# DINT-NSDI24/DINT

Hardware: AMD Instinct MI355X
Metric: Mtxn/s + p50/p99 batch latency, TATP (higher is better)
Workload: dtype u64

## Files before the change

### dint_amd/csrc/dint_kernels.h

```cpp
#pragma once
#include <hip/hip_runtime.h>
#include <stdint.h>

#include "dint_device.h"

struct dint_dev_stats {
  unsigned long long bad_requests;
  unsigned long long missing_keys;
  unsigned long long foreign_requests;
  unsigned long long pool_exhausted;
  unsigned long long route_overflow;
  unsigned long long big_bin_requests;
  unsigned long long late_requests;
  unsigned long long late_items[3];
};

struct dint_kv_sets {
  uint32_t *ctl[3] = {nullptr, nullptr, nullptr};
  uint32_t *pub[3] = {nullptr, nullptr, nullptr};
  uint32_t *bin_cnt[2] = {nullptr, nullptr};
  uint4 *kbins[2] = {nullptr, nullptr};
  uint4 *ovl[2] = {nullptr, nullptr};
  uint32_t *bigrdy = nullptr;
  uint64_t *sbx = nullptr;
  uint64_t pass_no = 0;
};

#define DINT_KV_HOTPUB_WORDS (3u * DINT_KV_BIGQ_MAX)
#define DINT_KV_SBX_WORDS 48u

struct dint_scratch {
  uint32_t *bin_cnt;
  uint64_t *bins;
  dint_dev_stats *stats;
  uint32_t *blk_cnt;
  uint32_t *blk_pub;
  uint32_t *blk_pub_next;
  uint32_t *big;
  uint32_t *big_next;
  uint32_t *bin_off;
  uint4 *ovl;
  uint64_t *ovf;
  uint64_t *ovf2;
  uint4 *kbins = nullptr;
  uint64_t kbins_slots = 0;
  uint4 *bigq = nullptr;
// ... 61 lines not shown
```

### dint_amd/csrc/dint_kv.h

```cpp
#pragma once
#include <cstdlib>
#include <utility>
#include <vector>

#include "dint_kernels.h"
#include "dint_kv_core.h"
#include "state_image.h"

#define DINT_KV_MAX_TABLES 5
#define DINT_KV_CTL_BYTES (64 + 24 * KV_NLISTS)
#define DINT_KV_TRACE_WORDS ((size_t)DINT_KV_PMAX * 16 + 16 * 8192)
#define DINT_KV_LOAD_OP 0xF0u

struct kv_dev {
  kv_tab tab[DINT_KV_MAX_TABLES];
  dint_mod mod[DINT_KV_MAX_TABLES];
  dint_mod lockmod[DINT_KV_MAX_TABLES];
  uint32_t gk_base[DINT_KV_MAX_TABLES];
  uint32_t n_tables;
  uint32_t shard_index, shard_count;
  uint32_t same_key;
};

struct dint_kv_knobs {
  uint32_t coarse_load = 512;
  uint32_t cap = 0;
  uint32_t lcap = 1024;
  uint32_t cap_mult = 64;
  uint32_t rpt = 0;
  uint32_t no_bm = 0;
  uint32_t hot_min = 0;
  uint32_t no_split = 0;
  uint32_t split_min = 65;
  uint32_t split_target = 384;
  uint32_t one_big_kernel = 0;
  uint32_t workers = 96;
  uint32_t part_first = 0;
  uint32_t sb_split_min = 65;
  uint32_t sb_npmax = 128;
  uint32_t sb_workers = 130;
  uint32_t sb_late_grid = 32;
  uint32_t residency = 0;
  uint32_t no_fuse = 0;
  uint32_t no_ahead = 0;
  uint32_t late_grid = 8;
  uint32_t exp_no_late = 0;
  uint32_t late_fat = 0;
  uint32_t late_big = 0;
};

struct dint_kv {
  uint32_t workload = 0;
  uint32_t n_tables = 0;
  uint32_t val_size = 0;
  int force_rounds = 0;
  uint64_t hash_size[DINT_KV_MAX_TABLES] = {0, 0, 0, 0, 0};
  kv_dev h{};
  kv_dev *d_dev = nullptr;
  uint8_t *d_ctl = nullptr;
  uint64_t *d_trace = nullptr;
  size_t entry_bytes[DINT_KV_MAX_TABLES] = {0, 0, 0, 0, 0};
  dint_kv_knobs knobs;
};

static inline uint32_t dint_kv_cap_mult() {
  const char *v = getenv("DINT_KV_CAP_MULT");
  const unsigned long m = v && *v ? strtoul(v, nullptr, 10) : 64ul;
  return (uint32_t)(m < 2 ? 2 : m > 256 ? 256 : m);
}
int dint_kv_create(dint_kv *kv, uint32_t workload, uint64_t n_rows, dint_shard shard, uint32_t pool_entries = 0,
// ... 135 lines not shown
```

### dint_amd/csrc/engine.hip

```cpp
#include <hip/hip_runtime.h>

#include <algorithm>
#include <cstdarg>
#include <cstdio>
#include <cstdlib>
#include <cstring>
#include <mutex>
#include <string>
#include <vector>

#include "../../include/dint_abi.h"
#include "dint_kernels.h"
#include "dint_kv.h"
#include "dint_populate.h"
#include "state_rehash.h"
#include "state_stats.h"

void dint_launch_lock_stage(uint32_t workload, int stage, const void *d_req, void *d_rep, uint32_t n, uint2 *table, dint_mod slots,
                            dint_shard shard, dint_scratch s, hipStream_t st, const dint_view &view);
bool dint_launch_lock_fused(uint32_t workload, void *d_rep, uint32_t n, uint2 *table, dint_mod slots, dint_shard shard, dint_scratch s,
                            const dint_view &view, const void *next_req, void *next_rep, uint32_t next_n, dint_scratch sn,
                            const dint_view &next_view, hipStream_t st);

namespace {
// ... 671 lines not shown
      TRY(dev_alloc((void **)&e->scratch.kvs.ovl[1], (size_t)e->pass_max * sizeof(uint4) * 2, false));
      TRY(dev_alloc((void **)&e->scratch.kvs.bigrdy, (size_t)DINT_KV_BIGQ_MAX * sizeof(uint32_t)));
      if (wl == DINT_WL_SMALLBANK)
        TRY(dev_alloc((void **)&e->scratch.kvs.sbx, (size_t)DINT_KV_BIGQ_MAX * DINT_KV_SBX_WORDS * sizeof(uint64_t), false));
    } else {
      TRY(dev_alloc((void **)&e->scratch.bins, (size_t)DINT_KV_PMAX * DINT_KV_BINCAP * sizeof(uint64_t), false));
      if (!getenv("DINT_LOCK_NO_DIRECT")) {
        e->scratch.kbins_slots = 1024ull * 65536ull;
        TRY(dev_alloc((void **)&e->scratch.kbins, (size_t)e->scratch.kbins_slots * sizeof(uint64_t), false));
      }
    }
    TRY(dev_alloc((void **)&e->scratch.blk_pub, 3 * 1024 * sizeof(uint32_t)));
    e->scratch.blk_pub_next = e->scratch.blk_pub + 1024;
    TRY(dev_alloc((void **)&e->scratch.big, 2 * (4 + DINT_KV_PMAX) * sizeof(uint32_t)));
    e->scratch.big_next = e->scratch.big + (4 + DINT_KV_PMAX);
    if (is_kv)
      for (int k = 0; k < 3; k++) { e->scratch.kvs.ctl[k] = e->scratch.big + 16 * k; e->scratch.kvs.pub[k] = e->scratch.blk_pub + 1024 * k; }
    TRY(dev_alloc((void **)&e->scratch.bin_off, DINT_KV_PMAX * sizeof(uint32_t)));
    TRY(hipMemset(e->scratch.bin_off, 0xFF, DINT_KV_PMAX * sizeof(uint32_t)) == hipSuccess ? 0 : fail(DINT_EHIP, "hipMemset"));
    TRY(dev_alloc((void **)&e->scratch.ovl, (size_t)e->pass_max * sizeof(uint4) * (is_kv ? 2 : 1), false));
    TRY(dev_alloc((void **)&e->scratch.ovf, (size_t)e->pass_max * sizeof(uint64_t), false));
    if (is_kv) {
      TRY(dev_alloc((void **)&e->scratch.ovf2, (size_t)e->pass_max * sizeof(uint64_t), false));
      e->scratch.kvs.bin_cnt[0] = e->scratch.bin_cnt; e->scratch.kvs.kbins[0] = e->scratch.kbins; e->scratch.kvs.ovl[0] = e->scratch.ovl;
    }
    if ((e->cfg.workload == DINT_WL_FASST || e->cfg.workload == DINT_WL_2PL) && getenv("DINT_KV_TRACE")) {
      TRY(dev_alloc((void **)&e->kv.d_trace, (size_t)DINT_KV_TRACE_WORDS * 8, true));
      e->scratch.lock_trace = e->kv.d_trace;
    }
  } else {
    TRY(dev_alloc((void **)&e->scratch.blk_pub, 2 * (1024 + 16) * sizeof(uint32_t)));
    e->scratch.blk_pub_next = e->scratch.blk_pub + (1024 + 16);
  }
  TRY(slot_alloc(e, 0));
  if (hipHostMalloc((void **)&e->h_pinned, (size_t)e->pass_max * e->msg_size + 64, hipHostMallocDefault) != hipSuccess ||
      hipHostMalloc((void **)&e->h_pool, 64, hipHostMallocDefault) != hipSuccess) {
    dint_engine_destroy(e);
    return fail(DINT_ENOMEM, "hipHostMalloc");
  }
  *e->h_pool = 0;

  if (wl == DINT_WL_FASST || wl == DINT_WL_2PL) {
    e->n_slots = cfg->n_slots ? cfg->n_slots : 36000000ull;
    if (e->n_slots > 0xFFFFFFF0ull) { dint_engine_destroy(e); return fail(DINT_EINVAL, "n_slots too large"); }
    e->slots_mod = dint_make_mod(e->n_slots);
    e->n_local_slots = (e->n_slots + e->shard.count - 1) / e->shard.count;
// ... 30 lines not shown
  for (auto &sl : e->slot)
    if (sl.deliver_to && sl.h_rep) { memcpy(sl.deliver_to, sl.h_rep, sl.deliver_bytes); sl.deliver_to = nullptr; }
  for (hipEvent_t ev : e->timer.ev) hipEventDestroy(ev);
  for (void *p : e->snap) hipFree(p);
  hipFree(e->scratch.bin_cnt);
  hipFree(e->scratch.bins);
  hipFree(e->scratch.kbins);
  hipFree(e->scratch.bigq);
  hipFree(e->scratch.hotpub);
  hipFree(e->scratch.lateq);
  hipFree(e->scratch.kvs.bin_cnt[1]);
  hipFree(e->scratch.kvs.kbins[1]);
  hipFree(e->scratch.kvs.ovl[1]);
  hipFree(e->scratch.kvs.bigrdy);
  hipFree(e->scratch.kvs.sbx);
  hipFree(e->scratch.stats);
  hipFree(e->scratch.blk_cnt);
  hipFree(std::min(e->scratch.blk_pub, e->scratch.blk_pub_next));
  hipFree(std::min(e->scratch.big, e->scratch.big_next));
  hipFree(e->scratch.bin_off);
  hipFree(e->scratch.ovl);
  hipFree(e->scratch.ovf);
  hipFree(e->scratch.ovf2);
  if (e->scratch.lock_trace) { hipFree(e->scratch.lock_trace); e->kv.d_trace = nullptr; }
  for (auto &sl : e->slot) {
    hipFree(sl.d_req);
    hipFree(sl.d_rep);
    if (sl.h_req) hipHostFree(sl.h_req);
    if (sl.h_rep) hipHostFree(sl.h_rep);
    if (sl.h2d) hipEventDestroy(sl.h2d);
    if (sl.comp) hipEventDestroy(sl.comp);
    if (sl.done) hipEventDestroy(sl.done);
  }
  hipFree(std::min(e->route.blk, e->route.blk_next));
  if (e->h_pinned) hipHostFree(e->h_pinned);
  if (e->h_pool) hipHostFree(e->h_pool);
  if (e->ev_order) hipEventDestroy(e->ev_order);
  if (e->ev_route_order) hipEventDestroy(e->ev_route_order);
  if (e->ev_wait) hipEventDestroy(e->ev_wait);
  if (e->ev_signal) hipEventDestroy(e->ev_signal);
  if (e->s_h2d && e->s_h2d != e->stream) hipStreamDestroy(e->s_h2d);
  if (e->s_d2h && e->s_d2h != e->stream) hipStreamDestroy(e->s_d2h);
  lock_pipe_destroy(e);
  replay_free(e);
  state_free(e);
  hipFree(e->tstats.part); hipFree(e->tstats.out);
// ... 1217 lines not shown
```

### dint_amd/csrc/k_kv.hip

```cpp
#include "k_kv_dev.h"

dint_kv_fmt dint_kv_format(uint32_t workload) {
  switch (workload) {
    case DINT_WL_STORE: return {53, 0, 0xFFFFFFFFu, 1, 9, 49, 40};
    case DINT_WL_TATP: return {55, 1, 2, 3, 11, 51, 40};
    default: return {23, 1, 2, 3, 11, 19, 8};
  }
}


static inline uint32_t kv_pick_coarse(uint32_t n, uint32_t load) {
  uint64_t c = ((uint64_t)n + load - 1) / load;
  if (c < 1) c = 1;
  if (c > DINT_KV_CMAX) c = DINT_KV_CMAX;
  return (uint32_t)c;
}
static uint32_t kv_env(const char *name, uint32_t dflt) {
  const char *v = getenv(name);
  return v && *v ? (uint32_t)strtoul(v, nullptr, 10) : dflt;
}
static dint_kv_knobs kv_read_knobs() {
  dint_kv_knobs k;
  k.coarse_load = std::min(8192u, std::max(64u, kv_env("DINT_KV_COARSE_LOAD", KVB_T)));
  k.cap = kv_env("DINT_KV_CAP", 0);
  k.lcap = std::min(KVR_LCAP, kv_env("DINT_KV_LCAP", KVR_LCAP));
  k.cap_mult = dint_kv_cap_mult();
  k.rpt = kv_env("DINT_KV_RPT", 0);
  k.no_bm = kv_env("DINT_KV_NO_BM", 0);
  k.hot_min = kv_env("DINT_KV_HOT_MIN", 0);
  k.no_split = kv_env("DINT_KV_NO_SPLIT", 0);
  k.split_min = std::max(65u, kv_env("DINT_KV_SPLIT_MIN", 65u));
  k.split_target = std::min(448u, std::max(8u, kv_env("DINT_KV_SPLIT_TARGET", 384u)));
  k.one_big_kernel = kv_env("DINT_KV_ONE_BIG_KERNEL", 0);
  k.no_ahead = kv_env("DINT_KV_NO_AHEAD", 0);
  k.no_fuse = kv_env("DINT_KV_NO_FUSE", 0);
  k.sb_split_min = kv_env("DINT_KV_SB_SPLIT_MIN", 65u);
  k.sb_late_grid = std::max(1u, std::min(KVB_GRID, kv_env("DINT_KV_SB_LATE_GRID", 32u)));
  k.sb_npmax = std::max(2u, std::min(KSB_NPMAX, kv_env("DINT_KV_SB_NPMAX", 128u)));
  k.sb_workers = kv_env("DINT_KV_SB_WORKERS", k.sb_npmax + 2u);
  if (k.sb_workers) k.sb_workers = std::max(k.sb_workers, k.sb_npmax + 2u);
  k.workers = std::min(1024u, std::max(KVR_NPMAX + 2u, kv_env("DINT_KV_WORKERS", KVW_GRID)));
  k.part_first = kv_env("DINT_KV_PART_FIRST", 0) & 1u;
  k.late_grid = std::min(KVB_GRID, std::max(1u, kv_env("DINT_KV_LATE_GRID", 8u)));
  k.late_big = kv_env("DINT_KV_LATE_BIG", 0);
  k.exp_no_late = kv_env("DINT_EXP_NO_LATE", 0);
  k.late_fat = kv_env("DINT_KV_LATE_FAT", 0);
  return k;
}

static inline bool kv_uses_hot(const dint_kv &kv, int load_mode) {
  return kv.workload != DINT_WL_SMALLBANK && !(kv.force_rounds & 3) && !load_mode && !kv.knobs.no_split;
}
bool dint_kv_one_launch(const dint_kv &kv, int load_mode) {
  return kv_uses_hot(kv, load_mode) && !kv.knobs.one_big_kernel && !kv.knobs.no_fuse;
}
bool dint_kv_ahead_ok(const dint_kv &kv, int load_mode) {
  if (kv.workload == DINT_WL_SMALLBANK) return !load_mode && !kv.knobs.no_ahead && !kv.knobs.no_fuse;
  return kv_uses_hot(kv, load_mode) && !kv.knobs.one_big_kernel && !kv.knobs.no_ahead;
}

static void kv_fill_pass(kv_pass_args &A, const void *d_req, void *d_rep, uint32_t n, const dint_kv &kv, dint_log log,
                         const dint_scratch &s, int load_mode, const dint_view &view, uint32_t tile) {
  const dint_kv_knobs &K = kv.knobs;
  const uint32_t C = kv_pick_coarse(n, K.coarse_load);
  const uint32_t mean = (n + C - 1) / C;
  uint32_t cap = K.cap_mult * mean + 64;
  cap = std::min(cap, (uint32_t)(s.kbins_slots / C));
  cap = std::max(1u, K.cap ? std::min(cap, K.cap) : cap);
  A.req = (const uint8_t *)d_req; A.rep = (uint8_t *)d_rep; A.n = n;
  A.n_tiles = (n + tile - 1) / tile;
  A.kv = kv.d_dev; A.log = log; A.cut = kv_make_cut(C, n); A.cap = cap;
  A.lcap = K.lcap;
  const uint64_t pn = s.kvs.pass_no;
  A.pno = (uint32_t)(pn & 1u);
  A.bin_cnt = s.kvs.bin_cnt[pn & 1]; A.kbins = s.kvs.kbins[pn & 1]; A.ovl = s.kvs.ovl[pn & 1];
  A.big = s.kvs.ctl[pn % 3]; A.big_z = s.kvs.ctl[(pn + 2) % 3];
  A.blk_pub = s.kvs.pub[pn % 3]; A.blk_pub_z = s.kvs.pub[(pn + 2) % 3];
  A.bigrdy = s.kvs.bigrdy;
  A.ovf = s.ovf; A.ovf2 = s.ovf2; A.stats = s.stats;
  A.bigq = s.bigq;
  A.hotpub = s.hotpub;
  A.lateq = s.lateq;
  A.seq = s.pass_seq ? s.pass_seq : 1u;
  A.inv_n = n > 1 ? (uint32_t)((1ull << 32) / n) : 0xFFFFFFFFu;
  A.load_mode = load_mode;
  A.force_flags = kv.force_rounds | (K.no_bm ? 4 : 0) | (int)(K.hot_min << 8);
  A.split_min = kv_uses_hot(kv, load_mode) ? K.split_min : 0xFFFFFFFFu;
  A.split_target = K.split_target;
  A.np_max = KVR_NPMAX;
  A.sb_pieces = 0;
  A.sbx = s.kvs.sbx;
  if (kv.workload == DINT_WL_SMALLBANK && K.sb_split_min && s.kvs.sbx && !(kv.force_rounds & 3) && !load_mode && !K.no_split) {
    A.split_min = std::max(8u, K.sb_split_min);
    A.np_max = K.sb_npmax;
    A.sb_pieces = 1;
  }
  A.has_log = kv.workload != DINT_WL_STORE;
  A.trace = kv.d_trace;
  A.V = view;
}

extern template int kv_piece_residency<DINT_WL_STORE>(int);
extern template int kv_piece_residency<DINT_WL_TATP>(int);
extern template int kv_piece_residency<DINT_WL_SMALLBANK>(int);
extern template void launch_kv_passes<DINT_WL_STORE>(kv_multi_args &, uint32_t, uint32_t, hipStream_t, hipEvent_t *, const dint_kv_knobs &, bool, const kv_multi_args *, uint32_t);
extern template void launch_kv_passes<DINT_WL_TATP>(kv_multi_args &, uint32_t, uint32_t, hipStream_t, hipEvent_t *, const dint_kv_knobs &, bool, const kv_multi_args *, uint32_t);
extern template void launch_kv_passes<DINT_WL_SMALLBANK>(kv_multi_args &, uint32_t, uint32_t, hipStream_t, hipEvent_t *, const dint_kv_knobs &, bool, const kv_multi_args *, uint32_t);

static inline uint32_t kv_pick_rpt(uint32_t n_total, const dint_kv_knobs &K) {
  if (K.rpt == 1 || K.rpt == 2 || K.rpt == 4) return K.rpt;
  return n_total >= 1024u * 1024u ? 4u : n_total >= 256u * 1024u ? 2u : 1u;
// ... 292 lines not shown
```

### dint_amd/csrc/k_kv_dev.h

```cpp
#pragma once
#include <algorithm>
#include <cstdlib>
#include <cstring>
#include <utility>
#include <vector>

#include "../../include/dint_abi.h"
#include "dint_kv.h"
#define KVB_SORT_INLINE
#include "dint_bins.h"

template <int WL> struct Fmt;
template <> struct Fmt<DINT_WL_STORE> {
  static constexpr uint32_t MSG = 53, TYPE = 0, KEY = 1, VAL = 9, VER = 49, VS = 40;
  static constexpr bool HAS_TABLE = false;
  static constexpr uint32_t TABLE = 0;
};
template <> struct Fmt<DINT_WL_TATP> {
  static constexpr uint32_t MSG = 55, TYPE = 1, KEY = 3, VAL = 11, VER = 51, VS = 40;
  static constexpr bool HAS_TABLE = true;
  static constexpr uint32_t TABLE = 2;
};
template <> struct Fmt<DINT_WL_SMALLBANK> {
  static constexpr uint32_t MSG = 23, TYPE = 1, KEY = 3, VAL = 11, VER = 19, VS = 8;
// ... 102 lines not shown
}

struct kv_pass_args {
  const uint8_t *req;
  uint8_t *rep;
  uint32_t n, n_tiles;
  const kv_dev *kv;
  dint_log log;
  kv_cut cut;
  uint32_t cap;
  uint32_t lcap;
  uint32_t *bin_cnt;
  uint4 *kbins;
  uint32_t *big, *big_z;
  uint32_t *blk_pub, *blk_pub_z;
  uint32_t *bigrdy;
  uint64_t *sbx;
  uint32_t np_max;
  uint32_t sb_pieces;
  uint32_t pno;
  uint4 *ovl;
  uint64_t *ovf;
  uint64_t *ovf2;
  uint4 *bigq;
  unsigned long long *hotpub;
  uint4 *lateq;
  uint32_t split_min;
  uint32_t split_target;
  uint32_t inv_n;
  uint32_t seq;
  dint_dev_stats *stats;
  int load_mode, force_flags;
  uint32_t has_log;
  uint64_t *trace;
  dint_view V;
};
struct kv_multi_args { kv_pass_args e[DINT_KV_MULTI_MAX]; };

__device__ static inline uint64_t u4_key(const uint4 &r) { return ((uint64_t)r.y << 32) | r.x; }
__device__ static inline uint64_t u4_meta(const uint4 &r) { return ((uint64_t)r.w << 32) | r.z; }

template <uint32_t TB, uint32_t... Ks>
__device__ __forceinline__ static void kv_copy_tile(const uint4 *__restrict__ s, uint4 *__restrict__ d, uint32_t nv, uint32_t t,
                                                    std::integer_sequence<uint32_t, Ks...>) {
  const uint4 v[] = {s[min(t + Ks * TB, nv - 1)]...};
  ((d[min(t + Ks * TB, nv - 1)] = v[Ks]), ...);
}

template <int RPT, uint32_t TB = KV_TB>
struct kv_part_lds {
  uint32_t Hc[DINT_KV_CMAX];
  uint32_t Sov[2];
  uint32_t Stile;
  uint32_t Swl[TB / 64 * RPT], Swp[TB / 64];
};
template <int WL, int RPT, uint32_t TB = KV_TB>
__device__ __forceinline__ static void kv_part_body(const kv_pass_args &A, kv_part_lds<RPT, TB> &S, bool first_block) {
  using F = Fmt<WL>;
  constexpr uint32_t T = TB * RPT, NWV = TB / 64;
  auto &Hc = S.Hc; auto &Sov = S.Sov; auto &Stile = S.Stile; auto &Swl = S.Swl; auto &Swp = S.Swp;
// ... 1884 lines not shown
#undef KVB_STAMP
}

#define KVR_LCAP 1024u
#define KVR_F 64u
#define KVR_NPMAX 64u
struct kvr_lds {
  uint4 rec[KVR_LCAP];
  uint32_t hist[KVR_F];
  uint32_t cur[KVR_F];
  uint32_t off[KVR_F + 1];
  uint32_t bigoff[KVR_F];
  uint2 chs[KVR_F];
  uint32_t nch;
  uint32_t cflag[KVR_F];
  uint64_t ckey[KVR_F], hrec[KVR_F];
};
__device__ static inline uint32_t kv_piece_of(uint32_t idx, uint32_t np, uint32_t inv_n) {
  const uint32_t p = (uint32_t)(((uint64_t)idx * np * inv_n) >> 32);
  return p < np ? p : np - 1;
}
#define KVQ_W 3u
enum : uint32_t { KVQ_SUB = 0, KVQ_PIECE = 1, KVQ_REM = 2, KVQ_SOLO = 3 };

__device__ static inline void kv_list_items(const kv_pass_args &A, uint32_t b, const kvr_lds &L, const uint2 *Sbig) {
  const uint32_t t = threadIdx.x & 63u;
  const uint2 bs = Sbig[t];
  uint32_t target = A.split_target;
  if (A.V.seg_cap) {
    uint32_t live = t < A.V.n_seg ? min(A.V.seg_cap, *(const uint32_t *)(A.V.cnt + (size_t)t * A.V.cnt_stride)) : 0u, tot;
    (void)wave_excl_scan_u32(live, &tot);
    if (tot < A.n) target = max(8u, (uint32_t)(((uint64_t)target * max(tot, 1u)) / A.n));
  }
  const uint32_t np0 = (bs.y + target - 1) / target;
  const bool hot = bs.y >= A.split_min && np0 <= A.np_max;
  const uint32_t np = hot ? np0 : 0u;
  const uint32_t nent = bs.y ? (np > 1 ? np + 1 : 1u) : 0u;
  uint32_t tot, at = wave_excl_scan_u32(nent, &tot);
  uint32_t base = 0;
  if (t == 0 && tot) base = atomicAdd(&A.big[3], tot);
  base = (uint32_t)__builtin_amdgcn_readfirstlane((int)base);
  at += base;
  const uint32_t bin = b + A.cut.P * t;
  if (nent && !hot) {
    kv_st_agent(A.bigq + KVQ_W * (size_t)at, make_uint4(bin, bs.x, bs.y, KVQ_SUB));
  } else if (nent) {
    uint64_t hk = L.ckey[t], hr = L.hrec[t];
    if (A.sb_pieces) {
      using F = Fmt<DINT_WL_SMALLBANK>;
      const uint32_t sh_g = 16 + A.cut.ibits;
      uint64_t smp[8];
#pragma unroll
      for (uint32_t j = 0; j < 8; j++) smp[j] = kv_ld_agent(&A.ovf[bs.x + (uint32_t)(((uint64_t)(2 * j + 1) * bs.y) >> 4)]);
      uint32_t best = 0, bj = 0;
#pragma unroll
      for (uint32_t j = 0; j < 8; j++) {
// ... 442 lines not shown
    for (uint32_t wv = 0; wv < KVB_W; wv++) {
      uint64_t mm = H.Bl[wv];
      if (wv * 64 > P) break;
      if (wv == (P >> 6)) mm &= (2ull << (P & 63)) - 1ull;
      if (mm) Gs = wv * 64 + 63 - (uint32_t)__clzll((long long)mm);
    }
    Ge = h;
    for (uint32_t wv = P >> 6; wv < KVB_W && Ge == h; wv++) {
      uint64_t mm = H.Bl[wv];
      if (wv == (P >> 6)) mm &= ~((2ull << (P & 63)) - 1ull);
      if (mm) Ge = wv * 64 + (uint32_t)__ffsll((unsigned long long)mm) - 1;
    }
  }
  auto rest = [&](uint32_t lo, uint32_t len) -> int {
    const uint32_t c_rem = h - len;
    if (c_rem == 0) return 0;
    __syncthreads();
    if (valid && (t < lo || t >= lo + len)) H.rem[t < lo ? t : t - len] = w;
    if (t >= c_rem) H.rem[t] = ~0ull;
    __builtin_amdgcn_fence(__ATOMIC_SEQ_CST, "workgroup");
    if (kv_rem_chunks<WL>(rep, cut2, kv, d.x, H.rem, c_rem, H, stats, force_rounds, V, true)) return 0;
    if (ovf2 && t < c_rem) {
      const uint64_t sw = H.rem[t];
      ovf2[d.y + t] = ((sw >> sh_g) << sh_g) | ((uint64_t)((uint32_t)(sw >> 7) & idx_mask) << 16) | ((uint32_t)sw & 0x7Fu) | (((uint32_t)(sw >> sh_k) & 511u) << 7);
    }
    __builtin_amdgcn_fence(__ATOMIC_SEQ_CST, "workgroup");
    *src = 1; *off = d.y; *cnt = c_rem;
    return 1;
  };
  auto phases = [&]() -> int {
    if (!kv_group_phases<WL>(rep, cut2, kv, d.x, H.all, Gs, Ge, H, stats, V)) return 1;
    return rest(Gs, Ge - Gs);
  };
  if (L <= 64) {
    if (ttr && t == 0) ttr[30] = (uint64_t)(d.w & 0xFFFFu) | (1ull << 17) | ((uint64_t)L << 20) | ((uint64_t)h << 32);
    if (Ge - Gs <= 64) return kv_rem_chunks<WL>(rep, cut2, kv, d.x, H.all, h, H, stats, force_rounds, V, true) ? 0 : 1;
    return phases();
  }
  const uint64_t hw = H.all[P];
  const uint32_t hq = pay_q((uint32_t)hw & 0x7Fu);
  const bool v = valid && t >= P && t < P + L;
  const uint32_t my_idx = (uint32_t)(w >> 7) & idx_mask, my_type = valid ? pay_type((uint32_t)w & 0x7Fu) : 0xFFu;
  if (valid && !v && (w >> sh_g) == (hw >> sh_g) && (kv_struct_op<WL>(my_type) || (kv_lock_op<WL>(my_type) && pay_q((uint32_t)w & 0x7Fu) == hq))) atomicOr(&H.bad, kv_struct_op<WL>(my_type) ? 1u : 2u);
  const uint64_t my_key = v ? ld_u64(rep + dint_view_off(V, my_idx, F::MSG) + F::KEY) : 0;
  if (t == P) H.hkey = my_key;
  const bool setop = v && is_set(my_type), insop = v && is_ins(my_type), delop = v && is_del(my_type);
  const bool lk = v && kv_lock_op<WL>(my_type), aq = v && WL == DINT_WL_TATP && my_type == 1;
// ... 154 lines not shown
    const bool same_g = k < h && (r >> sh_g) == (hrec >> sh_g), same = same_g && pay_kh(pay) == hkh;
    if (same_g && !same) {
      H.nbr = 1;
      if (kv_struct_op<WL>(type) || (kv_lock_op<WL>(type) && pay_q(pay) == hq)) H.bad = 1;
    }
    if (do_piece) {
      const bool mine = same && (np == 1 || kv_piece_of(ridx, np, inv_n) == j);
      const bool really = mine && ld_u64(rep + dint_view_off(V, ridx, F::MSG) + F::KEY) == hkey;
      if (mine && !really) H.bad = 1;
      const uint64_t mm = __ballot(really), ms = __ballot(same);
      uint32_t at = 0;
      if (lane == 0 && mm) at = atomicAdd(&H.nhot, (uint32_t)__popcll(mm));
      if (lane == 0 && ms) atomicAdd(&H.nsame, (uint32_t)__popcll(ms));
      at = (uint32_t)__builtin_amdgcn_readfirstlane((int)at) + (uint32_t)__popcll(mm & lanemask_lt());
      if (really && at < KVB_T) { H.key[at] = (ridx << 9) | at; H.typ[at] = (uint8_t)(type & 0xFFu); }
    }
    if (do_rem) {
      const bool other = k < h && !same;
      const uint64_t mm = __ballot(other);
      uint32_t at = 0;
      if (lane == 0 && mm) at = atomicAdd(&H.nrem, (uint32_t)__popcll(mm));
      at = (uint32_t)__builtin_amdgcn_readfirstlane((int)at) + (uint32_t)__popcll(mm & lanemask_lt());
      if (other) {
        ovf2[d.y + at] = r;
        if (at < KVB_T) H.rem[at] = r;
      }
    }
    if (solo && k < h && k < KVB_T) H.all[k] = r;
  }
  __syncthreads();
  const uint32_t c_rem = do_rem ? H.nrem : 0u, nbr = H.nbr;
  if (solo && H.nhot <= 64 && h <= KVB_T) {
    if (ttr && t == 0) ttr[30] = (uint64_t)(d.w & 0xFFFFu) | (1ull << 17) | ((uint64_t)H.nhot << 20) | ((uint64_t)h << 32);
    if (kv_rem_chunks<WL>(rep, cut2, kv, d.x, H.all, h, H, stats, force_rounds, V)) return 0;
    *src = 0; *off = d.y; *cnt = h;
    return 1;
  }
  const uint32_t c = do_piece ? H.nhot : 0u;
  if (t == 0 && c > KVB_T) H.bad = 1;
  const uint32_t nsib = np > 1 ? np + (nbr ? 1u : 0u) : 1u;
  const bool voting = do_piece || (nbr && np > 1);
  kv_hdr Hd;
  kv_tab tb0;
  uint64_t bucket0 = 0;
  uint32_t table0 = 0;
  const bool locator = t == 0 && c != 0;
  if (locator) {
// ... 128 lines not shown
        }
        st_u32(msg + F::VER, ver0 + nw_before + wr_below);
      }
      msg[F::TYPE] = (uint8_t)code;
    }
    if (found && nw_all && (int)j == jw && (int)t == lw_tot) {
      kv_copy_words(row, rep + dint_view_off(V, my_idx, F::MSG) + F::VAL, F::VS);
      KV_ST(uint32_t, &kv_entry_hdr(tb, bucket, H.link)->ver[H.slot], ver0 + nw_all);
    }
    if (WL == DINT_WL_TATP && t == 0) {
      if ((int)j == jl && la_fin >= 0 && (uint32_t)la_fin != la0) KV_ST(uint8_t, kv_entry_ptr(tb, bucket, KV_INLINE) + KV_LOCKB_OFF + hq, (uint8_t)la_fin);
      if (!found && wr_tot) atomicAdd(&stats->missing_keys, (unsigned long long)wr_tot);
    }
  }
  if (c_rem == 0) return 0;
  __builtin_amdgcn_fence(__ATOMIC_SEQ_CST, "workgroup");
  if (c_rem <= KVB_T && kv_rem_chunks<WL>(rep, cut2, kv, d.x, H.rem, c_rem, H, stats, force_rounds, V)) return 0;
  __builtin_amdgcn_fence(__ATOMIC_SEQ_CST, "workgroup");
  *src = 1; *off = d.y; *cnt = c_rem;
  return 1;
}

template <int WL>
__device__ __forceinline__ static void kv_serial_group(uint8_t *rep, const kv_cut cut2, const kv_dev *kv, uint32_t bin, const uint64_t *R, uint32_t Gs,
                                                       uint32_t Ge, kvh_lds &H, dint_dev_stats *__restrict__ stats, const dint_view V) {
  using F = Fmt<WL>;
  const uint32_t t = threadIdx.x, n = Ge - Gs;
  const uint32_t sh_g = 16 + cut2.ibits, idx_mask = (uint32_t)((1ull << cut2.ibits) - 1ull);
  __syncthreads();
  {
    const uint64_t w = t < n ? R[Gs + t] : 0;
    const uint32_t idx = (uint32_t)(w >> 7) & idx_mask, pay = (uint32_t)w & 0x7Fu;
    H.key[t] = t < n ? (idx << 9) | t : 0xFFFFFFFFu;
    H.typ[t] = (uint8_t)(pay_type(pay) & 0xFFu);
    H.qq[t] = (uint8_t)pay_q(pay);
  }
  __syncthreads();
  kvb_sort_blocked_u32<1>(H.key, KVB_T);
  if (t == 0) {
    const uint32_t gk = kv_cut_gk((uint32_t)(R[Gs] >> sh_g), bin, cut2), table = kv_table_of(kv, gk);
    const uint64_t bucket = (uint64_t)(gk - kv->gk_base[table]);
    for (uint32_t p = 0; p < n; p++) {
      const uint32_t sk = H.key[p], slot = sk & 511u;
      kv_do_request<WL>(rep + dint_view_off(V, sk >> 9, F::MSG), H.typ[slot], table, H.qq[slot], bucket, kv, stats);
      __builtin_amdgcn_fence(__ATOMIC_SEQ_CST, "workgroup");
    }
// ... 44 lines not shown
      return;
    }
    if (force_rounds || !kv_group_phases<WL>(rep, cut2, kv, bin, H.all, Gs, Gs + len, H, stats, V))
      kv_serial_group<WL>(rep, cut2, kv, bin, H.all, Gs, Gs + len, H, stats, V);
    __syncthreads();
    const bool mv = t >= Gs + len && t < m;
    const uint64_t mw = mv ? H.all[t] : 0;
    __syncthreads();
    if (mv) H.all[t - len] = mw;
    if (t >= m - len && t < m) H.all[t] = ~0ull;
    m -= len;
    if (m == 0) return;
  }
}
#define KVL_RANGES 4096u
struct kvl_lds {
  uint32_t pre[KVL_RANGES];
  uint32_t wsum[KVB_W];
  uint32_t cnt;
};
template <int WL>
__device__ __forceinline__ static void kv_late_item(const kv_pass_args &A, const kv_cut cut2, const kv_dev *kv, const uint4 d, kvh_lds &H, kvl_lds &L) {
  const uint32_t t = threadIdx.x, lane = t & 63, wave = t >> 6;
  const uint64_t *__restrict__ recs = (d.w ? (const uint64_t *)A.ovf2 : A.ovf) + d.y;
  const uint32_t cnt = d.z, bin = d.x;
  if (cnt == 0) return;
  if (cnt <= KVB_T) {
    __syncthreads();
    H.all[t] = t < cnt ? kv_sort_key(recs[t], cut2) : ~0ull;
    kv_late_stretch<WL>(A.rep, cut2, kv, bin, cnt, H, A.stats, A.force_flags & 1, A.V);
    return;
  }
  const uint32_t rw = (A.n + KVL_RANGES - 1) / KVL_RANGES;
  __syncthreads();
  for (uint32_t k = t; k < KVL_RANGES; k += KVB_T) L.pre[k] = 0;
  __syncthreads();
  for (uint32_t k = t; k < cnt; k += KVB_T) atomicAdd(&L.pre[min(KVL_RANGES - 1, kv_rec_idx(recs[k], cut2) / rw)], 1u);
  __syncthreads();
  {
    constexpr uint32_t PT = KVL_RANGES / KVB_T;
    uint32_t v[PT], sum = 0;
#pragma unroll
    for (uint32_t k = 0; k < PT; k++) { v[k] = L.pre[t * PT + k]; sum += v[k]; }
    uint32_t tot, base = wave_excl_scan_u32(sum, &tot);
    if (lane == 0) L.wsum[wave] = tot;
    __syncthreads();
    for (uint32_t w = 0; w < wave; w++) base += L.wsum[w];
// ... 315 lines not shown
      }
      st_u32(msg + F::VER, ver0 + nw_before + wr_below);
    } else if (get && my_type != 17u) {
      miss = 1;
    }
    msg[F::TYPE] = (uint8_t)code;
  }
  {
    const uint64_t mm = __ballot(miss != 0);
    if (lane == 0 && mm) atomicAdd(&stats->missing_keys, (unsigned long long)__popcll(mm));
  }
  if (found && nw_all && (int)j == jw && (int)t == lw_tot) {
    uint8_t *row = kv_entry_ptr(tb, bucket, H.link) + KV_VAL_OFF + H.slot * F::VS;
    KV_ST(uint32_t, row, ld_u32(msg + F::VAL));
    KV_ST(uint32_t, row + 4, ld_u32(msg + F::VAL + 4));
    KV_ST(uint32_t, &kv_entry_hdr(tb, bucket, H.link)->ver[H.slot], ver0 + nw_all);
  }
  return done();
}

static_assert(sizeof(kvb_lds) + KVB_BM_BYTES + sizeof(kv_dev) <= 160 * 1024, "k_kv_big must fit the 160 KB of LDS of a gfx950 CU");
static_assert(sizeof(kvb_lds) + (KV_HOT_BM ? KV_HOT_BM_W * 10 : 16) + sizeof(kv_dev) <= 160 * 1024, "k_kv_big must fit the 160 KB of LDS of a gfx950 CU");
#define KVW_GRID 96u
template <int WL>
__device__ __forceinline__ static void kv_hot_role(const kv_pass_args &A, kv_dev &Skv, uint8_t *Lraw, uint32_t &Stk, uint32_t bx, uint32_t by) {
  const uint32_t t = threadIdx.x;
  if (t < sizeof(kv_dev) / 4) ((uint32_t *)&Skv)[t] = ((const uint32_t *)A.kv)[t];
  __syncthreads();
  kv_dev_pend_set(Skv, A.pno);
  kv_cut cut2 = A.cut;
  cut2.P = A.cut.P * KVR_F;
  uint64_t *tr = A.trace ? A.trace + 2048 * 32 + 32 * (size_t)(by * KVB_GRID + bx) : nullptr;
  for (bool first = true;; first = false) {
    __syncthreads();
    if (t == 0) {
      const uint32_t i = atomicAdd(&A.big[4], 1u);
      uint32_t got = KV_NONE;
      for (uint32_t spins = 0; i < DINT_KV_BIGQ_MAX; spins++) {
        if (__hip_atomic_load(&A.bigrdy[i], __ATOMIC_RELAXED, __HIP_MEMORY_SCOPE_AGENT) == A.seq) { got = i; break; }
        if (__hip_atomic_load(&A.big[6], __ATOMIC_RELAXED, __HIP_MEMORY_SCOPE_AGENT) >= A.cut.P &&
            i >= __hip_atomic_load(&A.big[3], __ATOMIC_RELAXED, __HIP_MEMORY_SCOPE_AGENT)) break;
        if (spins > (1u << 22)) __builtin_trap();
        __builtin_amdgcn_s_sleep(4);
      }
      Stk = got;
    }
    __syncthreads();
    const uint32_t i = Stk;
    if (i == KV_NONE) break;
    const uint4 d = kv_ld_agent(A.bigq + KVQ_W * (size_t)i);
    uint32_t src = 0, off = d.y, cnt = d.z;
    uint64_t *ttr = first ? tr : nullptr;
    if (ttr && t == 0) { ttr[0] = __builtin_amdgcn_s_memrealtime(); ttr[2] = d.z; ttr[3] = d.x; ttr[30] = d.w; }
    int run = 1;
    if constexpr (WL == DINT_WL_SMALLBANK) {
      if ((d.w & 3u) != KVQ_SUB)
        run = kv_sb_item<WL>(A.rep, cut2, &Skv, d, kv_ld_agent(A.bigq + KVQ_W * (size_t)i + 1), kv_ld_agent(A.bigq + KVQ_W * (size_t)i + 2), A.ovf, A.ovf2,
                             A.hotpub, A.sbx, A.seq, A.inv_n, A.stats, A.V, Lraw, &src, &off, &cnt);
      if (run && src == 1 && cnt <= KVB_T) {
        kvh_lds &Hh = *(kvh_lds *)Lraw;
        __syncthreads();
        Hh.rem[t] = t < cnt ? A.ovf2[off + t] : 0ull;
        if (kv_rem_chunks<WL>(A.rep, cut2, &Skv, d.x, Hh.rem, cnt, Hh, A.stats, A.force_flags & 1, A.V)) run = 0;
      }
      if (run && t == 0) A.lateq[atomicAdd(&A.big[5], 1u)] = make_uint4(d.x, off, cnt, src);
    } else {
    if ((d.w & 3u) == KVQ_SOLO)
      run = kv_solo_item<WL>(A.rep, cut2, &Skv, d, A.ovf, A.ovf2, A.stats, A.force_flags & 1, A.V, Lraw, &src, &off, &cnt, ttr);
    else if ((d.w & 3u) != KVQ_SUB)
      run = kv_hot_item<WL>(A.rep, cut2, &Skv, d, kv_ld_agent(A.bigq + KVQ_W * (size_t)i + 1), kv_ld_agent(A.bigq + KVQ_W * (size_t)i + 2), A.ovf, A.ovf2,
                            A.hotpub, A.seq, A.inv_n, A.stats, A.force_flags & 1, A.V, Lraw, &src, &off, &cnt, ttr);
    if (run && t == 0) {
      A.lateq[atomicAdd(&A.big[5], 1u)] = make_uint4(d.x, off, cnt, src);
      atomicAdd(&A.stats->late_requests, (unsigned long long)cnt);
      atomicAdd(&A.stats->late_items[(d.w & 3u) == KVQ_SUB ? 0 : (d.w & 3u) == KVQ_SOLO ? 1 : 2], 1ULL);
    }
    }
    if (ttr && t == 0) ttr[1] = __builtin_amdgcn_s_memrealtime();
  }
}
template <int WL>
__global__ void __launch_bounds__(KVB_T, 4) k_kv_hot(kv_multi_args M) {
  __shared__ kv_dev Skv;
  __shared__ __attribute__((aligned(16))) uint8_t Lraw[sizeof(kvh_lds)];
  __shared__ uint32_t Stk;
  const kv_pass_args &A = M.e[blockIdx.y];
  if (blockIdx.x >= A.big[3]) return;
  kv_hot_role<WL>(A, Skv, Lraw, Stk, blockIdx.x, blockIdx.y);
}

template <int WL, int RPT>
__global__ void __launch_bounds__(KVB_T, 4) k_kv_hot_part(kv_pass_args H, kv_pass_args P) {
  constexpr size_t LB = sizeof(kvh_lds) > sizeof(kv_part_lds<RPT, KVB_T>) ? sizeof(kvh_lds) : sizeof(kv_part_lds<RPT, KVB_T>);
  __shared__ kv_dev Skv;
  __shared__ __attribute__((aligned(16))) uint8_t Lraw[LB];
  __shared__ uint32_t Stk;
  if (blockIdx.x < KVB_GRID) {
    if (blockIdx.x < H.big[3]) kv_hot_role<WL>(H, Skv, Lraw, Stk, blockIdx.x, 0);
    return;
// ... 9 lines not shown
                                                       uint32_t n_work ,
                                                       uint32_t part_first ) {
  constexpr size_t LW = sizeof(kvs_lds) > sizeof(kvh_lds) ? sizeof(kvs_lds) : sizeof(kvh_lds);
  constexpr size_t L1 = LW > sizeof(kvr_lds) ? LW : sizeof(kvr_lds);
  constexpr size_t LB = L1 > sizeof(kv_part_lds<RPT ? RPT : 1, KVB_T>) ? L1 : sizeof(kv_part_lds<RPT ? RPT : 1, KVB_T>);
  __shared__ kv_dev Skv;
  __shared__ __attribute__((aligned(16))) uint8_t Lraw[LB];
  __shared__ uint2 Sbig[KVR_F];
  __shared__ uint32_t Stk;
  uint32_t b = blockIdx.x;
  if (b < sum_c) {
    uint32_t e = 0;
    while (e + 1 < n_eng && b >= M.e[e].cut.P) { b -= M.e[e].cut.P; e++; }
    kv_resolve_role<WL>(M.e[e], b, Skv, Lraw, Sbig);
    return;
  }
  b -= sum_c;
  const uint32_t nw = n_work * n_eng, nt = RPT != 0 ? max_tiles * n_eng : 0u;
  const bool worker = part_first ? b >= nt : b < nw;
  if (worker) {
    if (part_first) b -= nt;
    if (b >= nw) return;
    const uint32_t e = b / n_work;
    kv_hot_role<WL>(M.e[e], Skv, Lraw, Stk, b - e * n_work, e);
    return;
  }
  if constexpr (RPT != 0) {
    if (!part_first) b -= nw;
    if (b >= nt) return;
    const uint32_t e = b / max_tiles, slot = b - e * max_tiles;
    const kv_pass_args &P = PM.e[e];
    if (slot >= P.n_tiles) return;
    kv_part_body<WL, RPT, KVB_T>(P, *(kv_part_lds<RPT, KVB_T> *)Lraw, slot == 0);
  }
}

template <int WL>
__global__ void __launch_bounds__(KVB_T, 1) k_kv_big(kv_multi_args M, uint32_t from_late) {
  static_assert(sizeof(kv_dev) + sizeof(kvb_lds) + (WL == DINT_WL_SMALLBANK ? KVB_BM_BYTES : 16) + 64 <= 160 * 1024, "k_kv_big's LDS must fit a gfx950 compute unit");
  __shared__ kv_dev Skv;
  __shared__ __attribute__((aligned(16))) uint8_t Lraw[sizeof(kvb_lds)];
  __shared__ __attribute__((aligned(16))) uint8_t Lbm[WL == DINT_WL_SMALLBANK ? KVB_BM_BYTES : KV_HOT_BM ? KV_HOT_BM_W * 10 : 16];
  __shared__ uint32_t Stk;
  const kv_pass_args &A = M.e[blockIdx.y];
  const uint32_t nq = from_late ? A.big[5] : A.big[3];
  if (blockIdx.x >= nq) return;
  const uint32_t t = threadIdx.x;
  if (t < sizeof(kv_dev) / 4) ((uint32_t *)&Skv)[t] = ((const uint32_t *)A.kv)[t];
  __syncthreads();
  kv_dev_pend_set(Skv, A.pno);
  __syncthreads();
  kv_cut cut2 = A.cut;
  cut2.P = A.cut.P * KVR_F;
  if (from_late) {
    for (uint32_t i = blockIdx.x; i < nq; i += gridDim.x) {
      const uint4 d = A.lateq[i];
      const uint64_t *recs = (d.w ? (const uint64_t *)A.ovf2 : A.ovf) + d.y;
      kv_big_bin<WL>(A.rep, A.n, cut2, &Skv, d.x, recs, d.w || !A.ovf2 ? nullptr : A.ovf2 + d.y, d.z, A.stats, A.force_flags, A.V, Lraw, Lbm, nullptr);
    }
    return;
  }
  uint64_t *tr = A.trace ? A.trace + 2048 * 32 + 32 * (size_t)(blockIdx.y * KVB_GRID + blockIdx.x) : nullptr;
  for (bool first = true;; first = false) {
    __syncthreads();
    if (t == 0) Stk = atomicAdd(&A.big[4], 1u);
    __syncthreads();
    const uint32_t i = Stk;
    if (i >= nq) break;
    const uint4 d = A.bigq[KVQ_W * (size_t)i];
    uint32_t src = 0, off = d.y, cnt = d.z;
    uint64_t *ttr = first ? tr : nullptr;
    if (ttr && t == 0) { ttr[0] = __builtin_amdgcn_s_memrealtime(); ttr[2] = d.z; ttr[3] = d.x; ttr[30] = d.w; }
    const uint64_t t_in = tr ? __builtin_amdgcn_s_memrealtime() : 0ull;
    int run = 1;
    if ((d.w & 3u) == KVQ_SOLO && WL != DINT_WL_SMALLBANK)
      run = kv_solo_item<WL>(A.rep, cut2, &Skv, d, A.ovf, A.ovf2, A.stats, A.force_flags & 1, A.V, Lraw, &src, &off, &cnt, ttr);
    else if ((d.w & 3u) != KVQ_SUB && WL == DINT_WL_SMALLBANK)
      run = kv_sb_item<WL>(A.rep, cut2, &Skv, d, A.bigq[KVQ_W * (size_t)i + 1], A.bigq[KVQ_W * (size_t)i + 2], A.ovf, A.ovf2, A.hotpub, A.sbx, A.seq,
                           A.inv_n, A.stats, A.V, Lraw, &src, &off, &cnt);
    else if ((d.w & 3u) != KVQ_SUB)
// ... 92 lines not shown
```

Baseline: 3059.

## Re-split leftover remainder records into a second level of hot pieces

When a hot-key piece leaves a remainder set (REM item), the worker now re-lists that remainder back onto the big queue as new pieces or a solo item instead of pushing it to the late queue. A third overflow buffer (ovf3) holds records from this second level, and a finish counter big[7] keeps workers from exiting while relisted items may still appear. The aim is to spread heavily contended bins across parallel workers rather than serialising them in the late pass. The cost is extra queue CAS traffic, a lane-0 heavy-hitter sampling loop, stronger agent-scope stores, and a more complex termination condition.

```diff
diff --git a/dint_amd/csrc/dint_kernels.h b/dint_amd/csrc/dint_kernels.h
--- a/dint_amd/csrc/dint_kernels.h
+++ b/dint_amd/csrc/dint_kernels.h
@@ -22,6 +22,7 @@
   uint4 *kbins[2] = {nullptr, nullptr};
   uint4 *ovl[2] = {nullptr, nullptr};
   uint32_t *bigrdy = nullptr;
+  uint64_t *ovf3 = nullptr;
   uint64_t *sbx = nullptr;
   uint64_t pass_no = 0;
 };
diff --git a/dint_amd/csrc/dint_kv.h b/dint_amd/csrc/dint_kv.h
--- a/dint_amd/csrc/dint_kv.h
+++ b/dint_amd/csrc/dint_kv.h
@@ -46,6 +46,7 @@
   uint32_t late_grid = 8;
   uint32_t exp_no_late = 0;
   uint32_t late_fat = 0;
+  uint32_t no_relist = 0;
   uint32_t late_big = 0;
 };
 
diff --git a/dint_amd/csrc/engine.hip b/dint_amd/csrc/engine.hip
--- a/dint_amd/csrc/engine.hip
+++ b/dint_amd/csrc/engine.hip
@@ -717,6 +717,7 @@
     TRY(dev_alloc((void **)&e->scratch.ovf, (size_t)e->pass_max * sizeof(uint64_t), false));
     if (is_kv) {
       TRY(dev_alloc((void **)&e->scratch.ovf2, (size_t)e->pass_max * sizeof(uint64_t), false));
+      if (wl != DINT_WL_SMALLBANK) TRY(dev_alloc((void **)&e->scratch.kvs.ovf3, (size_t)e->pass_max * sizeof(uint64_t), false));
       e->scratch.kvs.bin_cnt[0] = e->scratch.bin_cnt; e->scratch.kvs.kbins[0] = e->scratch.kbins; e->scratch.kvs.ovl[0] = e->scratch.ovl;
     }
     if ((e->cfg.workload == DINT_WL_FASST || e->cfg.workload == DINT_WL_2PL) && getenv("DINT_KV_TRACE")) {
@@ -793,6 +794,7 @@
   hipFree(e->scratch.ovl);
   hipFree(e->scratch.ovf);
   hipFree(e->scratch.ovf2);
+  hipFree(e->scratch.kvs.ovf3);
   if (e->scratch.lock_trace) { hipFree(e->scratch.lock_trace); e->kv.d_trace = nullptr; }
   for (auto &sl : e->slot) {
     hipFree(sl.d_req);
diff --git a/dint_amd/csrc/k_kv.hip b/dint_amd/csrc/k_kv.hip
--- a/dint_amd/csrc/k_kv.hip
+++ b/dint_amd/csrc/k_kv.hip
@@ -45,6 +45,7 @@
   k.late_big = kv_env("DINT_KV_LATE_BIG", 0);
   k.exp_no_late = kv_env("DINT_EXP_NO_LATE", 0);
   k.late_fat = kv_env("DINT_KV_LATE_FAT", 0);
+  k.no_relist = kv_env("DINT_KV_NO_RELIST", 0);
   return k;
 }
 
@@ -77,7 +78,7 @@
   A.big = s.kvs.ctl[pn % 3]; A.big_z = s.kvs.ctl[(pn + 2) % 3];
   A.blk_pub = s.kvs.pub[pn % 3]; A.blk_pub_z = s.kvs.pub[(pn + 2) % 3];
   A.bigrdy = s.kvs.bigrdy;
-  A.ovf = s.ovf; A.ovf2 = s.ovf2; A.stats = s.stats;
+  A.ovf = s.ovf; A.ovf2 = s.ovf2; A.ovf3 = s.kvs.ovf3; A.stats = s.stats;
   A.bigq = s.bigq;
   A.hotpub = s.hotpub;
   A.lateq = s.lateq;
@@ -87,6 +88,7 @@
   A.force_flags = kv.force_rounds | (K.no_bm ? 4 : 0) | (int)(K.hot_min << 8);
   A.split_min = kv_uses_hot(kv, load_mode) ? K.split_min : 0xFFFFFFFFu;
   A.split_target = K.split_target;
+  A.relist = kv_uses_hot(kv, load_mode) && !K.no_relist && s.kvs.ovf3 ? 1u : 0u;
   A.np_max = KVR_NPMAX;
   A.sb_pieces = 0;
   A.sbx = s.kvs.sbx;
diff --git a/dint_amd/csrc/k_kv_dev.h b/dint_amd/csrc/k_kv_dev.h
--- a/dint_amd/csrc/k_kv_dev.h
+++ b/dint_amd/csrc/k_kv_dev.h
@@ -148,9 +148,11 @@
   uint4 *ovl;
   uint64_t *ovf;
   uint64_t *ovf2;
+  uint64_t *ovf3;
   uint4 *bigq;
   unsigned long long *hotpub;
   uint4 *lateq;
+  uint32_t relist;
   uint32_t split_min;
   uint32_t split_target;
   uint32_t inv_n;
@@ -162,6 +164,7 @@
   dint_view V;
 };
 struct kv_multi_args { kv_pass_args e[DINT_KV_MULTI_MAX]; };
+static_assert(2 * sizeof(kv_multi_args) + 64 <= 4096, "k_kv_pass takes two of them: a kernel has 4 KB of arguments");
 
 __device__ static inline uint64_t u4_key(const uint4 &r) { return ((uint64_t)r.y << 32) | r.x; }
 __device__ static inline uint64_t u4_meta(const uint4 &r) { return ((uint64_t)r.w << 32) | r.z; }
@@ -2092,16 +2095,22 @@
 }
 #define KVQ_W 3u
 enum : uint32_t { KVQ_SUB = 0, KVQ_PIECE = 1, KVQ_REM = 2, KVQ_SOLO = 3 };
-
-__device__ static inline void kv_list_items(const kv_pass_args &A, uint32_t b, const kvr_lds &L, const uint2 *Sbig) {
+#define KVQ_L2 (1u << 18)
+
+__device__ static inline uint32_t kv_piece_target(const kv_pass_args &A) {
   const uint32_t t = threadIdx.x & 63u;
-  const uint2 bs = Sbig[t];
   uint32_t target = A.split_target;
   if (A.V.seg_cap) {
     uint32_t live = t < A.V.n_seg ? min(A.V.seg_cap, *(const uint32_t *)(A.V.cnt + (size_t)t * A.V.cnt_stride)) : 0u, tot;
     (void)wave_excl_scan_u32(live, &tot);
     if (tot < A.n) target = max(8u, (uint32_t)(((uint64_t)target * max(tot, 1u)) / A.n));
   }
+  return target;
+}
+__device__ static inline void kv_list_items(const kv_pass_args &A, uint32_t b, const kvr_lds &L, const uint2 *Sbig) {
+  const uint32_t t = threadIdx.x & 63u;
+  const uint2 bs = Sbig[t];
+  const uint32_t target = kv_piece_target(A);
   const uint32_t np0 = (bs.y + target - 1) / target;
   const bool hot = bs.y >= A.split_min && np0 <= A.np_max;
   const uint32_t np = hot ? np0 : 0u;
@@ -2590,7 +2599,7 @@
     if (kv_rem_chunks<WL>(rep, cut2, kv, d.x, H.rem, c_rem, H, stats, force_rounds, V, true)) return 0;
     if (ovf2 && t < c_rem) {
       const uint64_t sw = H.rem[t];
-      ovf2[d.y + t] = ((sw >> sh_g) << sh_g) | ((uint64_t)((uint32_t)(sw >> 7) & idx_mask) << 16) | ((uint32_t)sw & 0x7Fu) | (((uint32_t)(sw >> sh_k) & 511u) << 7);
+      kv_st_agent(&ovf2[d.y + t], ((sw >> sh_g) << sh_g) | ((uint64_t)((uint32_t)(sw >> 7) & idx_mask) << 16) | ((uint32_t)sw & 0x7Fu) | (((uint32_t)(sw >> sh_k) & 511u) << 7));
     }
     __builtin_amdgcn_fence(__ATOMIC_SEQ_CST, "workgroup");
     *src = 1; *off = d.y; *cnt = c_rem;
@@ -2791,7 +2800,7 @@
       if (lane == 0 && mm) at = atomicAdd(&H.nrem, (uint32_t)__popcll(mm));
       at = (uint32_t)__builtin_amdgcn_readfirstlane((int)at) + (uint32_t)__popcll(mm & lanemask_lt());
       if (other) {
-        ovf2[d.y + at] = r;
+        kv_st_agent(&ovf2[d.y + at], r);
         if (at < KVB_T) H.rem[at] = r;
       }
     }
@@ -2966,6 +2975,57 @@
 }
 
 template <int WL>
+__device__ __forceinline__ static bool kv_relist(const kv_pass_args &A, uint32_t bin, uint32_t off, uint32_t cnt) {
+  using F = Fmt<WL>;
+  const uint32_t lane = threadIdx.x & 63u;
+  const uint32_t target = kv_piece_target(A);
+  const uint32_t np = (cnt + target - 1) / target;
+  if (cnt == 0 || np > A.np_max) return false;
+  const uint32_t nent = np > 1 ? np + 1 : 1u;
+  uint32_t at = KV_NONE;
+  if (lane == 0) {
+    uint32_t cur = __hip_atomic_load(&A.big[3], __ATOMIC_RELAXED, __HIP_MEMORY_SCOPE_AGENT);
+    while (cur + nent <= DINT_KV_BIGQ_MAX) {
+      const uint32_t seen = atomicCAS(&A.big[3], cur, cur + nent);
+      if (seen == cur) { at = cur; break; }
+      cur = seen;
+    }
+  }
+  at = (uint32_t)__builtin_amdgcn_readfirstlane((int)at);
+  if (at == KV_NONE) return false;
+  uint64_t hk = 0, hr = 0;
+  if (np > 1) {
+    const uint32_t sh_g = 16 + A.cut.ibits;
+    if (lane == 0) {
+      uint32_t best = 0;
+#pragma clang loop unroll(disable)
+      for (uint32_t j = 0; j < 8; j++) {
+        const uint64_t sj = kv_ld_agent(&A.ovf2[off + (uint32_t)(((uint64_t)(2 * j + 1) * cnt) >> 4)]);
+        uint32_t c = 0;
+#pragma clang loop unroll(disable)
+        for (uint32_t i = 0; i < 8; i++) {
+          const uint64_t si = kv_ld_agent(&A.ovf2[off + (uint32_t)(((uint64_t)(2 * i + 1) * cnt) >> 4)]);
+          c += (si >> sh_g) == (sj >> sh_g) && pay_kh(kv_rec_pay(si)) == pay_kh(kv_rec_pay(sj)) ? 1u : 0u;
+        }
+        if (c > best) { best = c; hr = sj; }
+      }
+    }
+    hr = readlane_u64(hr, 0);
+    hk = ld_u64(A.rep + dint_view_off(A.V, kv_rec_idx(hr, A.cut), F::MSG) + F::KEY);
+  }
+  for (uint32_t p = lane; p < nent; p += 64) {
+    const uint32_t kind = np == 1 ? KVQ_SOLO : (p < np ? KVQ_PIECE : KVQ_REM);
+    uint4 *q = A.bigq + KVQ_W * (size_t)(at + p);
+    kv_st_agent(q, make_uint4(bin, off, cnt, kind | (p << 2) | (np << 10) | KVQ_L2));
+    kv_st_agent(q + 1, make_uint4((uint32_t)hk, (uint32_t)(hk >> 32), at, 0u));
+    kv_st_agent(q + 2, make_uint4((uint32_t)hr, (uint32_t)(hr >> 32), 0u, 0u));
+  }
+  asm volatile("s_waitcnt vmcnt(0)" ::: "memory");
+  for (uint32_t p = lane; p < nent; p += 64) __hip_atomic_store(&A.bigrdy[at + p], A.seq, __ATOMIC_RELAXED, __HIP_MEMORY_SCOPE_AGENT);
+  return true;
+}
+
+template <int WL>
 __device__ __forceinline__ static void kv_serial_group(uint8_t *rep, const kv_cut cut2, const kv_dev *kv, uint32_t bin, const uint64_t *R, uint32_t Gs,
                                                        uint32_t Ge, kvh_lds &H, dint_dev_stats *__restrict__ stats, const dint_view V) {
   using F = Fmt<WL>;
@@ -3056,7 +3116,7 @@
 template <int WL>
 __device__ __forceinline__ static void kv_late_item(const kv_pass_args &A, const kv_cut cut2, const kv_dev *kv, const uint4 d, kvh_lds &H, kvl_lds &L) {
   const uint32_t t = threadIdx.x, lane = t & 63, wave = t >> 6;
-  const uint64_t *__restrict__ recs = (d.w ? (const uint64_t *)A.ovf2 : A.ovf) + d.y;
+  const uint64_t *__restrict__ recs = (d.w == 2 ? (const uint64_t *)A.ovf3 : d.w ? (const uint64_t *)A.ovf2 : A.ovf) + d.y;
   const uint32_t cnt = d.z, bin = d.x;
   if (cnt == 0) return;
   if (cnt <= KVB_T) {
@@ -3418,7 +3478,7 @@
 static_assert(sizeof(kvb_lds) + KVB_BM_BYTES + sizeof(kv_dev) <= 160 * 1024, "k_kv_big must fit the 160 KB of LDS of a gfx950 CU");
 static_assert(sizeof(kvb_lds) + (KV_HOT_BM ? KV_HOT_BM_W * 10 : 16) + sizeof(kv_dev) <= 160 * 1024, "k_kv_big must fit the 160 KB of LDS of a gfx950 CU");
 #define KVW_GRID 96u
-template <int WL>
+template <int WL, bool RL = false >
 __device__ __forceinline__ static void kv_hot_role(const kv_pass_args &A, kv_dev &Skv, uint8_t *Lraw, uint32_t &Stk, uint32_t bx, uint32_t by) {
   const uint32_t t = threadIdx.x;
   if (t < sizeof(kv_dev) / 4) ((uint32_t *)&Skv)[t] = ((const uint32_t *)A.kv)[t];
@@ -3434,8 +3494,12 @@
       uint32_t got = KV_NONE;
       for (uint32_t spins = 0; i < DINT_KV_BIGQ_MAX; spins++) {
         if (__hip_atomic_load(&A.bigrdy[i], __ATOMIC_RELAXED, __HIP_MEMORY_SCOPE_AGENT) == A.seq) { got = i; break; }
-        if (__hip_atomic_load(&A.big[6], __ATOMIC_RELAXED, __HIP_MEMORY_SCOPE_AGENT) >= A.cut.P &&
-            i >= __hip_atomic_load(&A.big[3], __ATOMIC_RELAXED, __HIP_MEMORY_SCOPE_AGENT)) break;
+        if (__hip_atomic_load(&A.big[6], __ATOMIC_RELAXED, __HIP_MEMORY_SCOPE_AGENT) >= A.cut.P) {
+          const uint32_t fin = RL && A.relist ? __hip_atomic_load(&A.big[7], __ATOMIC_RELAXED, __HIP_MEMORY_SCOPE_AGENT) : 0xFFFFFFFFu;
+          asm volatile("s_waitcnt vmcnt(0)" ::: "memory");
+          const uint32_t listed = __hip_atomic_load(&A.big[3], __ATOMIC_RELAXED, __HIP_MEMORY_SCOPE_AGENT);
+          if (i >= listed && fin >= listed) break;
+        }
         if (spins > (1u << 22)) __builtin_trap();
         __builtin_amdgcn_s_sleep(4);
       }
@@ -3461,16 +3525,25 @@
       }
       if (run && t == 0) A.lateq[atomicAdd(&A.big[5], 1u)] = make_uint4(d.x, off, cnt, src);
     } else {
+    const bool l2 = RL && ((uint32_t)__builtin_amdgcn_readfirstlane((int)d.w) & KVQ_L2) != 0;
+    const uint64_t *rsrc = l2 ? (const uint64_t *)A.ovf2 : A.ovf;
+    uint64_t *rdst = l2 ? A.ovf3 : A.ovf2;
     if ((d.w & 3u) == KVQ_SOLO)
-      run = kv_solo_item<WL>(A.rep, cut2, &Skv, d, A.ovf, A.ovf2, A.stats, A.force_flags & 1, A.V, Lraw, &src, &off, &cnt, ttr);
+      run = kv_solo_item<WL>(A.rep, cut2, &Skv, d, rsrc, rdst, A.stats, A.force_flags & 1, A.V, Lraw, &src, &off, &cnt, ttr);
     else if ((d.w & 3u) != KVQ_SUB)
-      run = kv_hot_item<WL>(A.rep, cut2, &Skv, d, kv_ld_agent(A.bigq + KVQ_W * (size_t)i + 1), kv_ld_agent(A.bigq + KVQ_W * (size_t)i + 2), A.ovf, A.ovf2,
+      run = kv_hot_item<WL>(A.rep, cut2, &Skv, d, kv_ld_agent(A.bigq + KVQ_W * (size_t)i + 1), kv_ld_agent(A.bigq + KVQ_W * (size_t)i + 2), rsrc, rdst,
                             A.hotpub, A.seq, A.inv_n, A.stats, A.force_flags & 1, A.V, Lraw, &src, &off, &cnt, ttr);
+    if (RL && run && src == 1 && (d.w & (KVQ_L2 | 2u)) == 2u && A.relist) {
+      asm volatile("s_waitcnt vmcnt(0)" ::: "memory");
+      __syncthreads();
+      if (t < 64 && kv_relist<WL>(A, d.x, off, cnt)) run = 0;
+    }
     if (run && t == 0) {
-      A.lateq[atomicAdd(&A.big[5], 1u)] = make_uint4(d.x, off, cnt, src);
+      A.lateq[atomicAdd(&A.big[5], 1u)] = make_uint4(d.x, off, cnt, RL && (d.w & KVQ_L2) ? src + 1u : src);
       atomicAdd(&A.stats->late_requests, (unsigned long long)cnt);
       atomicAdd(&A.stats->late_items[(d.w & 3u) == KVQ_SUB ? 0 : (d.w & 3u) == KVQ_SOLO ? 1 : 2], 1ULL);
     }
+    if (RL && t == 0 && A.relist) atomicAdd(&A.big[7], 1u);
     }
     if (ttr && t == 0) ttr[1] = __builtin_amdgcn_s_memrealtime();
   }
@@ -3526,7 +3599,7 @@
     if (part_first) b -= nt;
     if (b >= nw) return;
     const uint32_t e = b / n_work;
-    kv_hot_role<WL>(M.e[e], Skv, Lraw, Stk, b - e * n_work, e);
+    kv_hot_role<WL, WL != DINT_WL_SMALLBANK>(M.e[e], Skv, Lraw, Stk, b - e * n_work, e);
     return;
   }
   if constexpr (RPT != 0) {
@@ -3559,7 +3632,7 @@
   if (from_late) {
     for (uint32_t i = blockIdx.x; i < nq; i += gridDim.x) {
       const uint4 d = A.lateq[i];
-      const uint64_t *recs = (d.w ? (const uint64_t *)A.ovf2 : A.ovf) + d.y;
+      const uint64_t *recs = (d.w == 2 ? (const uint64_t *)A.ovf3 : d.w ? (const uint64_t *)A.ovf2 : A.ovf) + d.y;
       kv_big_bin<WL>(A.rep, A.n, cut2, &Skv, d.x, recs, d.w || !A.ovf2 ? nullptr : A.ovf2 + d.y, d.z, A.stats, A.force_flags, A.V, Lraw, Lbm, nullptr);
     }
     return;
```

Result: slower. 2570 (-16.0%).
